# TorontoDeepLearning/convnet

Measured on AMD Instinct MI355X. Metric: images/sec (fprop+bprop+wgrad) AlexNet 224x224 bs=256, higher is better.
Workload: dtype f32

## Files before the change

convnet_amd/csrc/fewc_conv.hip:

```cpp
#include <algorithm>

#include "gather_gemm.h"

namespace chip {
namespace gfc {

constexpr int KX = 7, KY = 7, CH = 3, S = 2, NR = CH * KY, P = 4, IMG = 32;
constexpr int PW = S * (P - 1) + KX;
constexpr int XB = IMG * 4;
constexpr int RP = 2;
constexpr int ROWB = RP * 1024;
static_assert(PW * XB <= ROWB, "patch row");
constexpr int NCH = 10, ROWS = 96;
constexpr int H0_ROWS = 11, H1_ROWS = 10;
constexpr int H0_BYTES = H0_ROWS * ROWB, H1_BYTES = H1_ROWS * ROWB;
constexpr int BIAS_OFF = 0, BIAS_BYTES = 512;
constexpr int A_OFF = BIAS_BYTES;
constexpr int A_CHUNK = 6 * ROWS * 16;
constexpr int A_BYTES = NCH * A_CHUNK;
constexpr int A_PIECES = A_BYTES / 1024;
constexpr int PATCH_OFF = A_OFF + A_BYTES;
constexpr int ZERO_OFF = PATCH_OFF + H0_BYTES + H1_BYTES;
constexpr int ZERO_BYTES = 1024 + 256;
constexpr int LDS_BYTES = ZERO_OFF + ZERO_BYTES;
static_assert(LDS_BYTES <= 160 * 1024, "LDS");
static_assert(A_BYTES % 1024 == 0, "filter bank in whole pieces");
constexpr int NGROUP = 3 * 4;
constexpr int DUMP_BYTES = 4096;

__host__ __device__ constexpr int row_off(int r) { return r < 10 ? r * ROWB : r == 20 ? 10 * ROWB : H0_BYTES + (r - 10) * ROWB; }
__host__ __device__ constexpr int slot_k(int c, int lh, int j) {
  const int r = 2 * c + (j >> 2), kx = 2 * (j & 3) + lh;
  if (kx < KX) return kx + KX * r;
  return r < KX ? r + KX * 20 : -1;
}

struct Params {
  const float* src;
  const u32x4* planes;
  float* dst;
  float* dump;
  const float* bias;
  const float* zero;
  int F, N, H, W, My, Mx, pady, padx;
  int XG, IB, tiles;
  int relu;
  int diag;
};

}

__global__ void gfc_planes_kernel(const float* __restrict__ W, u32x4* __restrict__ out, int F) {
  using namespace gfc;
  const int i = blockIdx.x * blockDim.x + threadIdx.x;
  if (i >= NCH * 2 * ROWS) return;
  const int f = i % ROWS, lh = (i / ROWS) & 1, c = i / (2 * ROWS);
  Split8 sp = {};
  if (f < F) {
    float x[8];
#pragma unroll
    for (int j = 0; j < 8; ++j) {
      const int k = slot_k(c, lh, j);
      x[j] = k >= 0 ? W[(size_t)f + (size_t)F * k] : 0.f;
    }
    split8_sat(x, sp);
  }
  u32x4* o = out + ((size_t)c * 6 + lh) * ROWS + f;
  o[0] = sp.h;
  o[2 * ROWS] = sp.m;
  o[4 * ROWS] = sp.l;
}

template <bool RELU>
__global__ __launch_bounds__(320, 1) void gfc_kernel(const gfc::Params p) {
  using namespace gfc;
  extern __shared__ __attribute__((aligned(16))) float smem[];
  char* const lds = reinterpret_cast<char*>(smem);
  const int tid = threadIdx.x;
  const int wave = __builtin_amdgcn_readfirstlane(tid >> 6), lane = tid & 63;
  const int N = p.N;

  const int G = gridDim.x, q = p.tiles / G, rem = p.tiles % G, b = blockIdx.x;
  const int T0 = b * q + min(b, rem), T1 = T0 + q + (b < rem ? 1 : 0);
  if (T0 >= T1) return;
  int xg = T0 % p.XG, oy = (T0 / p.XG) % p.My, ib = T0 / (p.XG * p.My);
  auto next_tile = [&]() __attribute__((always_inline)) {
    if (++xg == p.XG) {
      xg = 0;
      if (++oy == p.My) {
        oy = 0;
        ++ib;
      }
    }
  };

  for (int i = wave; i < A_PIECES; i += 5) {
    const char* g = reinterpret_cast<const char*>(p.planes) + (size_t)i * 1024 + lane * 16;
    __builtin_amdgcn_global_load_lds((gbl_ptr_t)g, (lds_ptr_t)(lds + A_OFF + i * 1024), 16, 0, 0);
  }
  if (tid * 16 < ZERO_BYTES) *reinterpret_cast<u32x4*>(lds + ZERO_OFF + tid * 16) = u32x4{0, 0, 0, 0};
  if (tid < BIAS_BYTES / 4) *reinterpret_cast<float*>(lds + BIAS_OFF + tid * 4) = p.bias && tid < p.F ? p.bias[tid] : 0.f;

  if (wave == 4) {
    const int lx = lane >> 3;
    const unsigned lane_off = (unsigned)lx * (unsigned)(N * 4) + (unsigned)(lane & 7) * 16u;
    const size_t plane = (size_t)p.H * p.W * N * 4, rowb = (size_t)p.W * N * 4;
    auto issue_half = [&](auto HH) __attribute__((always_inline)) {
      constexpr int h = decltype(HH)::value;
      constexpr int n = h ? H1_ROWS : H0_ROWS;
      const int y0 = S * oy - p.pady, x0 = S * P * xg - p.padx;
      const char* const origin = reinterpret_cast<const char*>(p.src) + ((ptrdiff_t)y0 * p.W + x0) * (ptrdiff_t)(N * 4) + (ptrdiff_t)ib * (IMG * 4);
      bool xok[RP];
#pragma unroll
      for (int k = 0; k < RP; ++k) xok[k] = 8 * k + lx < PW && (unsigned)(x0 + 8 * k + lx) < (unsigned)p.W;
#pragma unroll
      for (int idx = 0; idx < n; ++idx) {
        const int r = h ? 10 + idx : idx == 10 ? 20 : idx;
        const int ch = r / KY, ky = r % KY;
        const bool yok = (unsigned)(y0 + ky) < (unsigned)p.H;
        const char* const rowp = origin + (size_t)ch * plane + (size_t)ky * rowb;
#pragma unroll
        for (int k = 0; k < RP; ++k) {
          const char* g = yok && xok[k] ? rowp + (size_t)(8 * k) * (size_t)(N * 4) + lane_off : reinterpret_cast<const char*>(p.zero);
          __builtin_amdgcn_global_load_lds((gbl_ptr_t)g, (lds_ptr_t)(lds + PATCH_OFF + (h ? H0_BYTES : 0) + idx * ROWB + k * 1024), 16, 0, 0);
        }
      }
    };
    using H0 = std::integral_constant<int, 0>;
    using H1 = std::integral_constant<int, 1>;
    issue_half(H0{});
    issue_half(H1{});
    __builtin_amdgcn_s_waitcnt(0x0070);
    __syncthreads();
    for (int T = T0; T < T1; ++T) {
      const bool more = T + 1 < T1 && !(p.diag & 2);
      __builtin_amdgcn_s_waitcnt(0x0070);
      __syncthreads();
      next_tile();
      if (more) issue_half(H0{});
      __builtin_amdgcn_s_waitcnt(0x0070);
      __syncthreads();
      if (more) issue_half(H1{});
    }
    __builtin_amdgcn_s_waitcnt(0x0070);
    return;
  }

  const int li = lane & 31, lh = lane >> 5;
  const unsigned base_l = (unsigned)(PATCH_OFF + (S * wave) * XB + li * 4 + lh * XB);
  const unsigned a_l = (unsigned)(A_OFF + (lh * ROWS + li) * 16);
  const unsigned lh_mask = lh ? 0xFFFFFFFFu : 0u;

  f32x16 acc[2][3];
  u32x4 fah[2][3], fam[3], fal[3];
  Split8 fb[2];
  float bv[8];
#ifndef CONVNET_EMU
#define CHIP_HERE() asm volatile("" ::: "memory")
#else
#define CHIP_HERE() ((void)0)
#endif
  auto read_a = [&](auto CC, auto PL, u32x4 (&dst)[3]) __attribute__((always_inline)) {
    constexpr int c = decltype(CC)::value, pl = decltype(PL)::value;
    CHIP_HERE();
#pragma unroll
    for (int t = 0; t < 3; ++t) dst[t] = *reinterpret_cast<const u32x4*>(lds + a_l + c * A_CHUNK + pl * (2 * ROWS * 16) + t * 512);
  };
  auto read_b = [&](auto CC) __attribute__((always_inline)) {
    constexpr int c = decltype(CC)::value;
    unsigned lhm = lh_mask;
    CHIP_HERE();
#ifndef CONVNET_EMU
    asm volatile("" : "+v"(lhm));
#endif
#pragma unroll
    for (int j = 0; j < 8; ++j) {
      const int r = 2 * c + (j >> 2);
      const int imm_n = row_off(r) + 2 * (j & 3) * XB;
      if ((j & 3) != 3) {
        bv[j] = *reinterpret_cast<const float*>(lds + base_l + imm_n);
      } else {
        const int imm_s = r < KX ? row_off(20) + (r - 1) * XB : (ZERO_OFF - PATCH_OFF);
        bv[j] = *reinterpret_cast<const float*>(lds + (base_l + (lhm & (unsigned)(imm_s - imm_n))) + imm_n);
      }
    }
  };
  auto split_pair = [&](int s, int q) __attribute__((always_inline)) {
    const float x0 = bv[2 * q], x1 = bv[2 * q + 1];
    const unsigned H = pk_bf16(x0, x1);
    const float r0 = x0 - __uint_as_float(H << 16), r1 = x1 - __uint_as_float(H & 0xffff0000u);
    const unsigned M = pk_bf16(r0, r1);
    const float s0 = r0 - __uint_as_float(M << 16), s1 = r1 - __uint_as_float(M & 0xffff0000u);
    fb[s].h[q] = H;
    fb[s].m[q] = M;
    fb[s].l[q] = pk_bf16(s0, s1);
#ifndef CONVNET_EMU
    asm volatile("" ::"v"(fb[s].h[q]), "v"(fb[s].m[q]), "v"(fb[s].l[q]));
#endif
  };
  auto mac_step = [&](auto K, int s, f32x16 (&a)[3]) __attribute__((always_inline)) {
    constexpr int k = decltype(K)::value;
#pragma unroll
    for (int t = 0; t < 3; ++t) {
      const u32x4& av = k == 1 ? fal[t] : k == 2 || k == 3 ? fam[t] : fah[s][t];
      const u32x4& bw = k == 0 ? fb[s].l : k == 2 || k == 4 ? fb[s].m : fb[s].h;
      a[t] = mma_bf16(av, bw, a[t]);
    }
#ifndef CONVNET_EMU
    asm volatile("" : "+v"(a[0]), "+v"(a[1]), "+v"(a[2]));
#endif
  };

  struct Out {
    unsigned lane_bytes;
    int flim;
  };
  const size_t fstride = (size_t)p.My * p.Mx * N;
  const int q4 = li & 3;
  auto out_of = [&](int xg_, int oy_, int ib_, bool exists) __attribute__((always_inline)) {
    const int ox = P * xg_ + wave;
    Out o;
    o.lane_bytes = (unsigned)((((size_t)oy_ * p.Mx + ox) * N + ib_ * IMG + 4 * (li >> 2) + (size_t)(q4 + 4 * lh) * fstride) * 4);
    o.flim = exists && ox < p.Mx ? p.F : 0;
#ifdef CONVNET_DIAG
    if (p.diag & 1) o.flim = 0;
#endif
    return o;
  };
  const unsigned bias_q = (unsigned)(BIAS_OFF + (q4 + 4 * lh) * 4);
  auto bias_of = [&](auto GG) __attribute__((always_inline)) {
    constexpr int gi = decltype(GG)::value;
    return *reinterpret_cast<const float*>(lds + bias_q + (32 * (gi >> 2) + 8 * (gi & 3)) * 4);
  };
  auto swap1 = [](float v) __attribute__((always_inline)) {
#ifndef CONVNET_EMU
    return __builtin_bit_cast(float, __builtin_amdgcn_mov_dpp(__builtin_bit_cast(int, v), 0xB1, 0xF, 0xF, true));
#else
    return emu::shfl_xor(v, 1);
#endif
  };
  auto swap2 = [](float v) __attribute__((always_inline)) {
#ifndef CONVNET_EMU
    return __builtin_bit_cast(float, __builtin_amdgcn_mov_dpp(__builtin_bit_cast(int, v), 0x4E, 0xF, 0xF, true));
#else
    return emu::shfl_xor(v, 2);
#endif
  };
  const bool odd1 = (li & 1) != 0, odd2 = (li & 2) != 0;
  auto store_group = [&](auto GG, const Out& o, const f32x16 (&a)[3], float bias) __attribute__((always_inline)) {
    constexpr int gi = decltype(GG)::value, t = gi >> 2, g = gi & 3;
    constexpr int cf = 32 * t + 8 * g;
    float x0 = a[t][4 * g], x1 = a[t][4 * g + 1], x2 = a[t][4 * g + 2], x3 = a[t][4 * g + 3];
    {
      const float r01 = swap1(odd1 ? x0 : x1), r23 = swap1(odd1 ? x2 : x3);
      x0 = odd1 ? r01 : x0; x1 = odd1 ? x1 : r01;
      x2 = odd1 ? r23 : x2; x3 = odd1 ? x3 : r23;
    }
    {
      const float ra = swap2(odd2 ? x0 : x2), rb = swap2(odd2 ? x1 : x3);
      x0 = odd2 ? ra : x0; x1 = odd2 ? rb : x1;
      x2 = odd2 ? x2 : ra; x3 = odd2 ? x3 : rb;
    }
    f32x4 v = {x0 + bias, x1 + bias, x2 + bias, x3 + bias};
    if constexpr (RELU) {
#pragma unroll
      for (int e = 0; e < 4; ++e) v[e] = fmaxf(v[e], 0.f);
    }
    const bool real = cf < o.flim;
    char* const rowb = real ? reinterpret_cast<char*>(p.dst) + (size_t)cf * fstride * 4 : reinterpret_cast<char*>(p.dump);
    const unsigned off = real ? o.lane_bytes : (unsigned)lane * 16u;
#ifdef CONVNET_DIAG
    if (p.diag & 4) return;
#endif
    *reinterpret_cast<f32x4*>(rowb + off) = v;
  };

  auto chunk_body = [&](auto CC, bool has_next, f32x16 (&cur)[3], const f32x16 (&prev)[3], const Out& po) __attribute__((always_inline)) {
    constexpr int c = decltype(CC)::value, s = c & 1;
    using CN = std::integral_constant<int, (c + 1) % NCH>;
    __builtin_amdgcn_sched_barrier(0);
    if (has_next) {
      read_b(CN{});
      read_a(CN{}, std::integral_constant<int, 0>{}, fah[s ^ 1]);
    }
    CHIP_HERE();
    const float bs0 = bias_of(std::integral_constant<int, c>{});
    float bs1 = 0.f;
    if constexpr (c >= 8) bs1 = bias_of(std::integral_constant<int, c + 2>{});
    static_for<0, 6>([&](auto KK) __attribute__((always_inline)) {
      constexpr int k = decltype(KK)::value;
      if constexpr (k >= 1 && k <= 4) {
        if (has_next) split_pair(s ^ 1, k - 1);
      }
      if constexpr (k == 0 && c >= 8) store_group(std::integral_constant<int, c + 2>{}, po, prev, bs1);
      if constexpr (k == 5) store_group(std::integral_constant<int, c>{}, po, prev, bs0);
      if constexpr (k == 2) {
        if (has_next) read_a(CN{}, std::integral_constant<int, 2>{}, fal);
      }
      if constexpr (k == 4) {
        if (has_next) read_a(CN{}, std::integral_constant<int, 1>{}, fam);
      }
      mac_step(KK, s, cur);
#pragma unroll
      for (int i = 0; i < 3; ++i) {
        __builtin_amdgcn_sched_group_barrier(0x008, 1, 0);
        __builtin_amdgcn_sched_group_barrier(0x100, 4, 0);
        __builtin_amdgcn_sched_group_barrier(0x002, 12, 0);
        __builtin_amdgcn_sched_group_barrier(0x040, 1, 0);
      }
      __builtin_amdgcn_sched_barrier(0);
    });
  };
  auto run_tile = [&](bool more, f32x16 (&cur)[3], const f32x16 (&prev)[3], const Out& po) __attribute__((always_inline)) {
#pragma unroll
    for (int t = 0; t < 3; ++t)
#pragma unroll
      for (int e = 0; e < 16; ++e) cur[t][e] = 0.f;
    static_for<0, NCH>([&](auto CC) __attribute__((always_inline)) {
      constexpr int c = decltype(CC)::value;
      if constexpr (c == 4) __syncthreads();
      if constexpr (c == NCH - 1) __syncthreads();
      if constexpr (c + 1 < NCH) chunk_body(CC, true, cur, prev, po);
      else chunk_body(CC, more, cur, prev, po);
    });
  };

  __builtin_amdgcn_s_waitcnt(0x0070);
  __syncthreads();
  {
    using C0 = std::integral_constant<int, 0>;
    read_b(C0{});
    read_a(C0{}, std::integral_constant<int, 0>{}, fah[0]);
    read_a(C0{}, std::integral_constant<int, 1>{}, fam);
    read_a(C0{}, std::integral_constant<int, 2>{}, fal);
  }
#pragma unroll
  for (int q4 = 0; q4 < 4; ++q4) split_pair(0, q4);
  Out po = out_of(0, 0, 0, false);
  int T = T0;
  for (;;) {
    run_tile(T + 1 < T1, acc[0], acc[1], po);
    po = out_of(xg, oy, ib, true);
    next_tile();
    if (++T >= T1) {
      static_for<0, NGROUP>([&](auto GG) __attribute__((always_inline)) { store_group(GG, po, acc[0], bias_of(GG)); });
      break;
    }
    run_tile(T + 1 < T1, acc[1], acc[0], po);
    po = out_of(xg, oy, ib, true);
    next_tile();
    if (++T >= T1) {
      static_for<0, NGROUP>([&](auto GG) __attribute__((always_inline)) { store_group(GG, po, acc[1], bias_of(GG)); });
      break;
    }
  }
}

bool gfc_try(const float* images, const float* filters, const float* bias, float* targets, int N, int C, int H, int W, int F, int Ky, int Kx,
             int sy, int sx, int pady, int padx, int My, int Mx, float scaleTargets, int relu, double flops) {
  using namespace gfc;
  if (!CHIP_KNOB("CONVNET_GG_FEWC", 1) || matrix_path() != 1) return false;
  if (Kx != KX || Ky != KY || C != CH || sy != S || sx != S || F > ROWS || F < 8 || F % 8 != 0 || N % IMG != 0 || My < 1 || Mx < 1) return false;
  if (pady < 0 || padx < 0 || (size_t)C * H * W * N * 4 >= (size_t(1) << 32) || (size_t)F * My * Mx * N * 4 >= (size_t(1) << 32)) return false;
  if (scaleTargets != 0.f) return false;
  if ((reinterpret_cast<uintptr_t>(images) | reinterpret_cast<uintptr_t>(targets)) & 15) return false;
  static bool once = false;
  static int cus = 256;
  if (!once) {
    CHIP_CHECK(hipFuncSetAttribute(reinterpret_cast<const void*>(gfc_kernel<false>), hipFuncAttributeMaxDynamicSharedMemorySize, LDS_BYTES));
    CHIP_CHECK(hipFuncSetAttribute(reinterpret_cast<const void*>(gfc_kernel<true>), hipFuncAttributeMaxDynamicSharedMemorySize, LDS_BYTES));
#ifndef CONVNET_EMU
    int dev = 0;
    hipDeviceProp_t prop;
    if (hipGetDevice(&dev) == hipSuccess && hipGetDeviceProperties(&prop, dev) == hipSuccess && prop.multiProcessorCount > 0) cus = prop.multiProcessorCount;
#else
    cus = 4;
#endif
    once = true;
  }
  u32x4* planes = static_cast<u32x4*>(workspace_aux(A_BYTES + DUMP_BYTES));
  (void)filter_planes_shared(nullptr, 0);
  {
    KernelTimer timer("filter_planes_kernel", "conv_fprop", 0.0, 4.0 * F * C * Ky * Kx + A_BYTES);
    hipLaunchKernelGGL(gfc_planes_kernel, dim3(divup(NCH * 2 * ROWS, 256)), dim3(256), 0, stream(), filters, planes, F);
  }
  Params p{};
  p.src = images; p.planes = planes; p.dst = targets; p.bias = bias; p.zero = zero_page();
  p.dump = reinterpret_cast<float*>(reinterpret_cast<char*>(planes) + A_BYTES);
  p.F = F; p.N = N; p.H = H; p.W = W; p.My = My; p.Mx = Mx; p.pady = pady; p.padx = padx;
  p.XG = divup(Mx, P); p.IB = N / IMG; p.tiles = p.XG * My * p.IB;
  p.relu = relu; p.diag = CHIP_DIAG_KNOB("CONVNET_GFC_DIAG", 0);
  const int grid = std::min(cus, p.tiles);
  {
    KernelTimer timer("gfc_kernel<96x128,split>", "conv_fprop", flops, 0.0, 0.0);
    if (relu) hipLaunchKernelGGL(gfc_kernel<true>, dim3(grid), dim3(320), LDS_BYTES, stream(), p);
    else hipLaunchKernelGGL(gfc_kernel<false>, dim3(grid), dim3(320), LDS_BYTES, stream(), p);
  }
  note_kernel("gfc_kernel(fprop)", flops, grid, 1);
  return true;
}

}
```

Baseline: 27920.

## Add wide 8-pixel tile variant for first-layer conv with shared producer loads

Adds a WIDE variant of the few-channel 7x7 stride-2 conv kernel in which each wave computes two output pixels, so there are 8 per tile instead of 4. Overlapping input columns are reused by shifting the already-split bf16 halves rather than re-splitting them. The dedicated producer wave is removed; all four compute waves share the patch refill and wait on vmcnt so that stores can stay in flight. Accumulators are pinned to AGPRs and the first MMA starts from a zero accumulator. The wide path is chosen when there are at least four tiles per CU, which costs more LDS and register pressure.

Measured after the change: 28000 (median of 3 runs). No clear change (+0.3%).

```diff
diff --git a/convnet_amd/csrc/fewc_conv.hip b/convnet_amd/csrc/fewc_conv.hip
--- a/convnet_amd/csrc/fewc_conv.hip
+++ b/convnet_amd/csrc/fewc_conv.hip
@@ -5,30 +5,48 @@
 namespace chip {
 namespace gfc {
 
-constexpr int KX = 7, KY = 7, CH = 3, S = 2, NR = CH * KY, P = 4, IMG = 32;
-constexpr int PW = S * (P - 1) + KX;
+constexpr int KX = 7, KY = 7, CH = 3, S = 2, NR = CH * KY, IMG = 32;
 constexpr int XB = IMG * 4;
-constexpr int RP = 2;
-constexpr int ROWB = RP * 1024;
-static_assert(PW * XB <= ROWB, "patch row");
 constexpr int NCH = 10, ROWS = 96;
 constexpr int H0_ROWS = 11, H1_ROWS = 10;
-constexpr int H0_BYTES = H0_ROWS * ROWB, H1_BYTES = H1_ROWS * ROWB;
 constexpr int BIAS_OFF = 0, BIAS_BYTES = 512;
 constexpr int A_OFF = BIAS_BYTES;
 constexpr int A_CHUNK = 6 * ROWS * 16;
 constexpr int A_BYTES = NCH * A_CHUNK;
 constexpr int A_PIECES = A_BYTES / 1024;
 constexpr int PATCH_OFF = A_OFF + A_BYTES;
-constexpr int ZERO_OFF = PATCH_OFF + H0_BYTES + H1_BYTES;
 constexpr int ZERO_BYTES = 1024 + 256;
-constexpr int LDS_BYTES = ZERO_OFF + ZERO_BYTES;
-static_assert(LDS_BYTES <= 160 * 1024, "LDS");
 static_assert(A_BYTES % 1024 == 0, "filter bank in whole pieces");
-constexpr int NGROUP = 3 * 4;
 constexpr int DUMP_BYTES = 4096;
 
-__host__ __device__ constexpr int row_off(int r) { return r < 10 ? r * ROWB : r == 20 ? 10 * ROWB : H0_BYTES + (r - 10) * ROWB; }
+template <bool WIDE>
+struct Tile {
+  static constexpr int P = WIDE ? 8 : 4;
+  static constexpr int PPW = P / 4;
+  static constexpr int PW = S * (P - 1) + KX;
+  static constexpr int RP = WIDE ? 3 : 2;
+  static constexpr int ROWB = RP * 1024;
+  static constexpr int H0_BYTES = H0_ROWS * ROWB, H1_BYTES = H1_ROWS * ROWB;
+  static constexpr int ZERO_OFF = PATCH_OFF + H0_BYTES + H1_BYTES;
+  static constexpr int LDS_BYTES = ZERO_OFF + ZERO_BYTES;
+  static constexpr int THREADS = WIDE ? 256 : 320;
+  static constexpr int NACC = 3 * PPW;
+  static constexpr int NGROUP = 4 * NACC;
+  static_assert(PW * XB <= ROWB, "patch row");
+  static_assert(LDS_BYTES <= 160 * 1024, "LDS");
+  static_assert((WIDE ? 0 : S * 3 * XB) + (PPW - 1) * S * XB + XB + IMG * 4 <= ZERO_BYTES, "zero region");
+  __host__ __device__ static constexpr int row_off(int r) { return r < 10 ? r * ROWB : r == 20 ? 10 * ROWB : H0_BYTES + (r - 10) * ROWB; }
+};
+__host__ __device__ constexpr int wide_extra(int c) { return c == 1 ? 0 : c == 3 ? 1 : c == 6 ? 2 : c == 8 ? 3 : -1; }
+__host__ __device__ constexpr int wide_stores(int c0, int n) {
+  int s = 0;
+  for (int i = 0; i < n; ++i) s += 2 + (wide_extra((c0 + i) % NCH) >= 0 ? 1 : 0);
+  return s;
+}
+static_assert(wide_stores(0, NCH) == Tile<true>::NGROUP, "every group of the previous tile leaves during this one");
+constexpr int WIDE_STORES_IN_FLIGHT = wide_stores(4, 5);
+static_assert(wide_stores(9, 5) == WIDE_STORES_IN_FLIGHT && WIDE_STORES_IN_FLIGHT < 16, "one vmcnt immediate for both refill waits");
+
 __host__ __device__ constexpr int slot_k(int c, int lh, int j) {
   const int r = 2 * c + (j >> 2), kx = 2 * (j & 3) + lh;
   if (kx < KX) return kx + KX * r;
@@ -71,9 +89,12 @@
   o[4 * ROWS] = sp.l;
 }
 
-template <bool RELU>
-__global__ __launch_bounds__(320, 1) void gfc_kernel(const gfc::Params p) {
+template <bool RELU, bool WIDE>
+__global__ __launch_bounds__(gfc::Tile<WIDE>::THREADS, 1) void gfc_kernel(const gfc::Params p) {
   using namespace gfc;
+  using TL = Tile<WIDE>;
+  constexpr int P = TL::P, PPW = TL::PPW, PW = TL::PW, RP = TL::RP, ROWB = TL::ROWB, H0_BYTES = TL::H0_BYTES, ZERO_OFF = TL::ZERO_OFF;
+  constexpr int NACC = TL::NACC, NGROUP = TL::NGROUP, NW = TL::THREADS / 64;
   extern __shared__ __attribute__((aligned(16))) float smem[];
   char* const lds = reinterpret_cast<char*>(smem);
   const int tid = threadIdx.x;
@@ -94,67 +115,131 @@
     }
   };
 
-  for (int i = wave; i < A_PIECES; i += 5) {
+  for (int i = wave; i < A_PIECES; i += NW) {
     const char* g = reinterpret_cast<const char*>(p.planes) + (size_t)i * 1024 + lane * 16;
     __builtin_amdgcn_global_load_lds((gbl_ptr_t)g, (lds_ptr_t)(lds + A_OFF + i * 1024), 16, 0, 0);
   }
   if (tid * 16 < ZERO_BYTES) *reinterpret_cast<u32x4*>(lds + ZERO_OFF + tid * 16) = u32x4{0, 0, 0, 0};
   if (tid < BIAS_BYTES / 4) *reinterpret_cast<float*>(lds + BIAS_OFF + tid * 4) = p.bias && tid < p.F ? p.bias[tid] : 0.f;
 
-  if (wave == 4) {
-    const int lx = lane >> 3;
-    const unsigned lane_off = (unsigned)lx * (unsigned)(N * 4) + (unsigned)(lane & 7) * 16u;
-    const size_t plane = (size_t)p.H * p.W * N * 4, rowb = (size_t)p.W * N * 4;
-    auto issue_half = [&](auto HH) __attribute__((always_inline)) {
-      constexpr int h = decltype(HH)::value;
-      constexpr int n = h ? H1_ROWS : H0_ROWS;
-      const int y0 = S * oy - p.pady, x0 = S * P * xg - p.padx;
-      const char* const origin = reinterpret_cast<const char*>(p.src) + ((ptrdiff_t)y0 * p.W + x0) * (ptrdiff_t)(N * 4) + (ptrdiff_t)ib * (IMG * 4);
-      bool xok[RP];
-#pragma unroll
-      for (int k = 0; k < RP; ++k) xok[k] = 8 * k + lx < PW && (unsigned)(x0 + 8 * k + lx) < (unsigned)p.W;
-#pragma unroll
-      for (int idx = 0; idx < n; ++idx) {
-        const int r = h ? 10 + idx : idx == 10 ? 20 : idx;
-        const int ch = r / KY, ky = r % KY;
-        const bool yok = (unsigned)(y0 + ky) < (unsigned)p.H;
-        const char* const rowp = origin + (size_t)ch * plane + (size_t)ky * rowb;
-#pragma unroll
-        for (int k = 0; k < RP; ++k) {
-          const char* g = yok && xok[k] ? rowp + (size_t)(8 * k) * (size_t)(N * 4) + lane_off : reinterpret_cast<const char*>(p.zero);
-          __builtin_amdgcn_global_load_lds((gbl_ptr_t)g, (lds_ptr_t)(lds + PATCH_OFF + (h ? H0_BYTES : 0) + idx * ROWB + k * 1024), 16, 0, 0);
-        }
-      }
-    };
-    using H0 = std::integral_constant<int, 0>;
-    using H1 = std::integral_constant<int, 1>;
-    issue_half(H0{});
-    issue_half(H1{});
-    __builtin_amdgcn_s_waitcnt(0x0070);
-    __syncthreads();
-    for (int T = T0; T < T1; ++T) {
-      const bool more = T + 1 < T1 && !(p.diag & 2);
+  const int lx = lane >> 3;
+  const unsigned lane_off = (unsigned)lx * (unsigned)(N * 4) + (unsigned)(lane & 7) * 16u;
+  const size_t plane = (size_t)p.H * p.W * N * 4, rowb = (size_t)p.W * N * 4;
+  struct RowSrc {
+    size_t rel;
+    int ky;
+  };
+  auto row_src = [&](int h, int idx) __attribute__((always_inline)) {
+    const int r = h ? 10 + idx : idx == 10 ? 20 : idx;
+    const int ch = r / KY, ky = r % KY;
+    return RowSrc{(size_t)ch * plane + (size_t)ky * rowb, ky};
+  };
+  struct Origin {
+    const char* at;
+    int y0;
+    bool xok[RP];
+  };
+  auto origin_of = [&](int xg_, int oy_, int ib_) __attribute__((always_inline)) {
+    Origin o;
+    const int x0 = S * P * xg_ - p.padx;
+    o.y0 = S * oy_ - p.pady;
+    o.at = reinterpret_cast<const char*>(p.src) + ((ptrdiff_t)o.y0 * p.W + x0) * (ptrdiff_t)(N * 4) + (ptrdiff_t)ib_ * (IMG * 4);
+#pragma unroll
+    for (int k = 0; k < RP; ++k) o.xok[k] = 8 * k + lx < PW && (unsigned)(x0 + 8 * k + lx) < (unsigned)p.W;
+    return o;
+  };
+  auto issue_row = [&](auto HH, int idx, const RowSrc& rs, const Origin& o) __attribute__((always_inline)) {
+    constexpr int h = decltype(HH)::value;
+    const bool yok = (unsigned)(o.y0 + rs.ky) < (unsigned)p.H;
+    const char* const rowp = o.at + rs.rel;
+#pragma unroll
+    for (int k = 0; k < RP; ++k) {
+      const char* g = yok && o.xok[k] ? rowp + (size_t)(8 * k) * (size_t)(N * 4) + lane_off : reinterpret_cast<const char*>(p.zero);
+      __builtin_amdgcn_global_load_lds((gbl_ptr_t)g, (lds_ptr_t)(lds + PATCH_OFF + (h ? H0_BYTES : 0) + idx * ROWB + k * 1024), 16, 0, 0);
+    }
+  };
+  using H0 = std::integral_constant<int, 0>;
+  using H1 = std::integral_constant<int, 1>;
+
+  if constexpr (!WIDE) {
+    if (wave == 4) {
+      auto issue_half = [&](auto HH) __attribute__((always_inline)) {
+        constexpr int h = decltype(HH)::value;
+        const Origin o = origin_of(xg, oy, ib);
+#pragma unroll
+        for (int idx = 0; idx < (h ? H1_ROWS : H0_ROWS); ++idx) issue_row(HH, idx, row_src(h, idx), o);
+      };
+      issue_half(H0{});
+      issue_half(H1{});
       __builtin_amdgcn_s_waitcnt(0x0070);
       __syncthreads();
-      next_tile();
-      if (more) issue_half(H0{});
+      for (int T = T0; T < T1; ++T) {
+        const bool more = T + 1 < T1 && !(p.diag & 2);
+        __builtin_amdgcn_s_waitcnt(0x0070);
+        __syncthreads();
+        next_tile();
+        if (more) issue_half(H0{});
+        __builtin_amdgcn_s_waitcnt(0x0070);
+        __syncthreads();
+        if (more) issue_half(H1{});
+      }
       __builtin_amdgcn_s_waitcnt(0x0070);
-      __syncthreads();
-      if (more) issue_half(H1{});
-    }
-    __builtin_amdgcn_s_waitcnt(0x0070);
-    return;
+      return;
+    }
+  }
+  constexpr int NSHARE = 3;
+  static_assert(!WIDE || (4 * NSHARE >= H0_ROWS && 4 * (NSHARE - 1) < H1_ROWS), "rows of a half over four waves");
+  RowSrc share_src[2][NSHARE];
+  if constexpr (WIDE) {
+#pragma unroll
+    for (int h = 0; h < 2; ++h)
+#pragma unroll
+      for (int m = 0; m < NSHARE; ++m) share_src[h][m] = row_src(h, min(wave + 4 * m, (h ? H1_ROWS : H0_ROWS) - 1));
+  }
+  auto issue_share = [&](auto HH, int xg_, int oy_, int ib_) __attribute__((always_inline)) {
+    constexpr int h = decltype(HH)::value;
+    const Origin o = origin_of(xg_, oy_, ib_);
+#pragma unroll
+    for (int m = 0; m < NSHARE; ++m) {
+      const int idx = wave + 4 * m;
+      if (m + 1 < NSHARE || idx < (h ? H1_ROWS : H0_ROWS)) issue_row(HH, idx, share_src[h][m], o);
+    }
+  };
+  int nxg = 0, noy = 0, nib = 0;
+  auto peek_next = [&]() __attribute__((always_inline)) {
+    nxg = xg; noy = oy; nib = ib;
+    if (++nxg == p.XG) {
+      nxg = 0;
+      if (++noy == p.My) {
+        noy = 0;
+        ++nib;
+      }
+    }
+  };
+  auto wait_refill = [&]() __attribute__((always_inline)) {
+#ifdef CONVNET_DIAG
+    if (p.diag & 4) {
+      __builtin_amdgcn_s_waitcnt(0x0070);
+      return;
+    }
+#endif
+    __builtin_amdgcn_s_waitcnt(0x0070 | WIDE_STORES_IN_FLIGHT);
+  };
+  if constexpr (WIDE) {
+    issue_share(H0{}, xg, oy, ib);
+    issue_share(H1{}, xg, oy, ib);
   }
 
   const int li = lane & 31, lh = lane >> 5;
-  const unsigned base_l = (unsigned)(PATCH_OFF + (S * wave) * XB + li * 4 + lh * XB);
+  const unsigned base_l = (unsigned)(PATCH_OFF + (S * PPW * wave) * XB + li * 4 + lh * XB);
   const unsigned a_l = (unsigned)(A_OFF + (lh * ROWS + li) * 16);
   const unsigned lh_mask = lh ? 0xFFFFFFFFu : 0u;
-
-  f32x16 acc[2][3];
+  const unsigned zero_rel = (unsigned)(ZERO_OFF - PATCH_OFF) - (unsigned)((S * PPW * wave) * XB);
+
+  f32x16 acc[2][NACC];
   u32x4 fah[2][3], fam[3], fal[3];
-  Split8 fb[2];
-  float bv[8];
+  Split8 fb[2][PPW];
+  float bv[PPW][8];
 #ifndef CONVNET_EMU
 #define CHIP_HERE() asm volatile("" ::: "memory")
 #else
@@ -176,60 +261,92 @@
 #pragma unroll
     for (int j = 0; j < 8; ++j) {
       const int r = 2 * c + (j >> 2);
-      const int imm_n = row_off(r) + 2 * (j & 3) * XB;
-      if ((j & 3) != 3) {
-        bv[j] = *reinterpret_cast<const float*>(lds + base_l + imm_n);
-      } else {
-        const int imm_s = r < KX ? row_off(20) + (r - 1) * XB : (ZERO_OFF - PATCH_OFF);
-        bv[j] = *reinterpret_cast<const float*>(lds + (base_l + (lhm & (unsigned)(imm_s - imm_n))) + imm_n);
-      }
-    }
-  };
-  auto split_pair = [&](int s, int q) __attribute__((always_inline)) {
-    const float x0 = bv[2 * q], x1 = bv[2 * q + 1];
+      const int imm_n = TL::row_off(r) + 2 * (j & 3) * XB;
+      unsigned at = base_l;
+      if ((j & 3) == 3) {
+        if (WIDE && r >= KX) {
+          at = base_l + (lhm & (zero_rel - (unsigned)imm_n));
+        } else {
+          const int imm_s = r < KX ? TL::row_off(20) + (r - 1) * XB : (ZERO_OFF - PATCH_OFF);
+          at = base_l + (lhm & (unsigned)(imm_s - imm_n));
+        }
+      }
+#pragma unroll
+      for (int px = 0; px < PPW; ++px)
+        if (px == 0 || (j & 3) >= 2) bv[px][j] = *reinterpret_cast<const float*>(lds + at + imm_n + px * (S * XB));
+    }
+  };
+  auto split_pair = [&](int s, int px, int q) __attribute__((always_inline)) {
+    if (px > 0 && (q & 1) == 0) {
+      const Split8& f0 = fb[s][px - 1];
+      Split8& f = fb[s][px];
+      f.h[q] = (f0.h[q] >> 16) | (f0.h[q + 1] << 16);
+      f.m[q] = (f0.m[q] >> 16) | (f0.m[q + 1] << 16);
+      f.l[q] = (f0.l[q] >> 16) | (f0.l[q + 1] << 16);
+#ifndef CONVNET_EMU
+      asm volatile("" ::"v"(f.h[q]), "v"(f.m[q]), "v"(f.l[q]));
+#endif
+      return;
+    }
+    const float x0 = bv[px][2 * q], x1 = bv[px][2 * q + 1];
     const unsigned H = pk_bf16(x0, x1);
     const float r0 = x0 - __uint_as_float(H << 16), r1 = x1 - __uint_as_float(H & 0xffff0000u);
     const unsigned M = pk_bf16(r0, r1);
     const float s0 = r0 - __uint_as_float(M << 16), s1 = r1 - __uint_as_float(M & 0xffff0000u);
-    fb[s].h[q] = H;
-    fb[s].m[q] = M;
-    fb[s].l[q] = pk_bf16(s0, s1);
-#ifndef CONVNET_EMU
-    asm volatile("" ::"v"(fb[s].h[q]), "v"(fb[s].m[q]), "v"(fb[s].l[q]));
-#endif
-  };
-  auto mac_step = [&](auto K, int s, f32x16 (&a)[3]) __attribute__((always_inline)) {
+    Split8& f = fb[s][px];
+    f.h[q] = H;
+    f.m[q] = M;
+    f.l[q] = pk_bf16(s0, s1);
+#ifndef CONVNET_EMU
+    asm volatile("" ::"v"(f.h[q]), "v"(f.m[q]), "v"(f.l[q]));
+#endif
+  };
+  auto mac_step = [&](auto K, auto FIRST, int s, f32x16 (&a)[NACC]) __attribute__((always_inline)) {
     constexpr int k = decltype(K)::value;
-#pragma unroll
-    for (int t = 0; t < 3; ++t) {
-      const u32x4& av = k == 1 ? fal[t] : k == 2 || k == 3 ? fam[t] : fah[s][t];
-      const u32x4& bw = k == 0 ? fb[s].l : k == 2 || k == 4 ? fb[s].m : fb[s].h;
-      a[t] = mma_bf16(av, bw, a[t]);
-    }
-#ifndef CONVNET_EMU
-    asm volatile("" : "+v"(a[0]), "+v"(a[1]), "+v"(a[2]));
+    constexpr bool first = decltype(FIRST)::value;
+#pragma unroll
+    for (int px = 0; px < PPW; ++px) {
+#pragma unroll
+      for (int t = 0; t < 3; ++t) {
+        const u32x4& av = k == 1 ? fal[t] : k == 2 || k == 3 ? fam[t] : fah[s][t];
+        const Split8& f = fb[s][px];
+        const u32x4& bw = k == 0 ? f.l : k == 2 || k == 4 ? f.m : f.h;
+        if constexpr (first) {
+          const f32x16 zero = {0.f, 0.f, 0.f, 0.f, 0.f, 0.f, 0.f, 0.f, 0.f, 0.f, 0.f, 0.f, 0.f, 0.f, 0.f, 0.f};
+          a[3 * px + t] = mma_bf16(av, bw, zero);
+        } else {
+          a[3 * px + t] = mma_bf16(av, bw, a[3 * px + t]);
+        }
+      }
+    }
+#ifndef CONVNET_EMU
+    if constexpr (WIDE) asm volatile("" : "+a"(a[0]), "+a"(a[1]), "+a"(a[2]), "+a"(a[3]), "+a"(a[4]), "+a"(a[5]));
+    else asm volatile("" : "+v"(a[0]), "+v"(a[1]), "+v"(a[2]));
 #endif
   };
 
   struct Out {
-    unsigned lane_bytes;
-    int flim;
+    unsigned lane_bytes[PPW];
+    int flim[PPW];
   };
   const size_t fstride = (size_t)p.My * p.Mx * N;
   const int q4 = li & 3;
   auto out_of = [&](int xg_, int oy_, int ib_, bool exists) __attribute__((always_inline)) {
-    const int ox = P * xg_ + wave;
     Out o;
-    o.lane_bytes = (unsigned)((((size_t)oy_ * p.Mx + ox) * N + ib_ * IMG + 4 * (li >> 2) + (size_t)(q4 + 4 * lh) * fstride) * 4);
-    o.flim = exists && ox < p.Mx ? p.F : 0;
+#pragma unroll
+    for (int px = 0; px < PPW; ++px) {
+      const int ox = P * xg_ + PPW * wave + px;
+      o.lane_bytes[px] = (unsigned)((((size_t)oy_ * p.Mx + ox) * N + ib_ * IMG + 4 * (li >> 2) + (size_t)(q4 + 4 * lh) * fstride) * 4);
+      o.flim[px] = exists && ox < p.Mx ? p.F : 0;
 #ifdef CONVNET_DIAG
-    if (p.diag & 1) o.flim = 0;
-#endif
+      if (p.diag & 1) o.flim[px] = 0;
+#endif
+    }
     return o;
   };
   const unsigned bias_q = (unsigned)(BIAS_OFF + (q4 + 4 * lh) * 4);
   auto bias_of = [&](auto GG) __attribute__((always_inline)) {
-    constexpr int gi = decltype(GG)::value;
+    constexpr int gi = decltype(GG)::value % 12;
     return *reinterpret_cast<const float*>(lds + bias_q + (32 * (gi >> 2) + 8 * (gi & 3)) * 4);
   };
   auto swap1 = [](float v) __attribute__((always_inline)) {
@@ -247,10 +364,11 @@
 #endif
   };
   const bool odd1 = (li & 1) != 0, odd2 = (li & 2) != 0;
-  auto store_group = [&](auto GG, const Out& o, const f32x16 (&a)[3], float bias) __attribute__((always_inline)) {
-    constexpr int gi = decltype(GG)::value, t = gi >> 2, g = gi & 3;
+  auto store_group = [&](auto GG, const Out& o, const f32x16 (&a)[NACC], float bias) __attribute__((always_inline)) {
+    constexpr int gi = decltype(GG)::value, px = gi / 12, t = (gi % 12) >> 2, g = gi & 3;
     constexpr int cf = 32 * t + 8 * g;
-    float x0 = a[t][4 * g], x1 = a[t][4 * g + 1], x2 = a[t][4 * g + 2], x3 = a[t][4 * g + 3];
+    const f32x16& at = a[3 * px + t];
+    float x0 = acc_elem<WIDE>(at[4 * g]), x1 = acc_elem<WIDE>(at[4 * g + 1]), x2 = acc_elem<WIDE>(at[4 * g + 2]), x3 = acc_elem<WIDE>(at[4 * g + 3]);
     {
       const float r01 = swap1(odd1 ? x0 : x1), r23 = swap1(odd1 ? x2 : x3);
       x0 = odd1 ? r01 : x0; x1 = odd1 ? x1 : r01;
@@ -266,16 +384,16 @@
 #pragma unroll
       for (int e = 0; e < 4; ++e) v[e] = fmaxf(v[e], 0.f);
     }
-    const bool real = cf < o.flim;
+    const bool real = cf < o.flim[px];
     char* const rowb = real ? reinterpret_cast<char*>(p.dst) + (size_t)cf * fstride * 4 : reinterpret_cast<char*>(p.dump);
-    const unsigned off = real ? o.lane_bytes : (unsigned)lane * 16u;
+    const unsigned off = real ? o.lane_bytes[px] : (unsigned)lane * 16u;
 #ifdef CONVNET_DIAG
     if (p.diag & 4) return;
 #endif
     *reinterpret_cast<f32x4*>(rowb + off) = v;
   };
 
-  auto chunk_body = [&](auto CC, bool has_next, f32x16 (&cur)[3], const f32x16 (&prev)[3], const Out& po) __attribute__((always_inline)) {
+  auto chunk_body = [&](auto CC, bool has_next, f32x16 (&cur)[NACC], const f32x16 (&prev)[NACC], const Out& po) __attribute__((always_inline)) {
     constexpr int c = decltype(CC)::value, s = c & 1;
     using CN = std::integral_constant<int, (c + 1) % NCH>;
     __builtin_amdgcn_sched_barrier(0);
@@ -284,42 +402,75 @@
       read_a(CN{}, std::integral_constant<int, 0>{}, fah[s ^ 1]);
     }
     CHIP_HERE();
-    const float bs0 = bias_of(std::integral_constant<int, c>{});
-    float bs1 = 0.f;
-    if constexpr (c >= 8) bs1 = bias_of(std::integral_constant<int, c + 2>{});
+    constexpr int G0 = WIDE ? (wide_extra(c) >= 0 ? 2 * NCH + wide_extra(c) : -1) : (c >= 8 ? c + 2 : -1);
+    constexpr int G3 = WIDE ? 2 * c : -1, G5 = WIDE ? 2 * c + 1 : c;
+    const float bs5 = bias_of(std::integral_constant<int, G5>{});
+    float bs0 = 0.f, bs3 = 0.f;
+    if constexpr (G0 >= 0) bs0 = bias_of(std::integral_constant<int, G0>{});
+    if constexpr (G3 >= 0) bs3 = bias_of(std::integral_constant<int, G3>{});
     static_for<0, 6>([&](auto KK) __attribute__((always_inline)) {
       constexpr int k = decltype(KK)::value;
-      if constexpr (k >= 1 && k <= 4) {
-        if (has_next) split_pair(s ^ 1, k - 1);
-      }
-      if constexpr (k == 0 && c >= 8) store_group(std::integral_constant<int, c + 2>{}, po, prev, bs1);
-      if constexpr (k == 5) store_group(std::integral_constant<int, c>{}, po, prev, bs0);
+      if constexpr (!WIDE) {
+        if constexpr (k >= 1 && k <= 4) {
+          if (has_next) split_pair(s ^ 1, 0, k - 1);
+        }
+      } else {
+        constexpr int i0 = k == 1 ? 0 : k == 2 ? 3 : k == 4 ? 6 : 8, i1 = k == 1 ? 3 : k == 2 ? 6 : 8;
+        if (has_next) {
+#pragma unroll
+          for (int i = i0; i < i1; ++i) split_pair(s ^ 1, i >> 2, i & 3);
+        }
+      }
+      if constexpr (k == 0 && G0 >= 0) store_group(std::integral_constant<int, (G0 >= 0 ? G0 : 0)>{}, po, prev, bs0);
+      if constexpr (k == 3 && G3 >= 0) store_group(std::integral_constant<int, (G3 >= 0 ? G3 : 0)>{}, po, prev, bs3);
+      if constexpr (k == 5) store_group(std::integral_constant<int, G5>{}, po, prev, bs5);
       if constexpr (k == 2) {
         if (has_next) read_a(CN{}, std::integral_constant<int, 2>{}, fal);
       }
       if constexpr (k == 4) {
         if (has_next) read_a(CN{}, std::integral_constant<int, 1>{}, fam);
       }
-      mac_step(KK, s, cur);
-#pragma unroll
-      for (int i = 0; i < 3; ++i) {
+      mac_step(KK, std::bool_constant<WIDE && c == 0 && k == 0>{}, s, cur);
+#pragma unroll
+      for (int i = 0; i < NACC; ++i) {
         __builtin_amdgcn_sched_group_barrier(0x008, 1, 0);
         __builtin_amdgcn_sched_group_barrier(0x100, 4, 0);
-        __builtin_amdgcn_sched_group_barrier(0x002, 12, 0);
+        __builtin_amdgcn_sched_group_barrier(0x002, WIDE ? 8 : 12, 0);
         __builtin_amdgcn_sched_group_barrier(0x040, 1, 0);
       }
       __builtin_amdgcn_sched_barrier(0);
     });
   };
-  auto run_tile = [&](bool more, f32x16 (&cur)[3], const f32x16 (&prev)[3], const Out& po) __attribute__((always_inline)) {
-#pragma unroll
-    for (int t = 0; t < 3; ++t)
-#pragma unroll
-      for (int e = 0; e < 16; ++e) cur[t][e] = 0.f;
+  auto run_tile = [&](bool more, f32x16 (&cur)[NACC], const f32x16 (&prev)[NACC], const Out& po) __attribute__((always_inline)) {
+    if constexpr (!WIDE) {
+#pragma unroll
+      for (int t = 0; t < 3; ++t)
+#pragma unroll
+        for (int e = 0; e < 16; ++e) cur[t][e] = 0.f;
+    }
+    const bool refill = more && !(p.diag & 2);
     static_for<0, NCH>([&](auto CC) __attribute__((always_inline)) {
       constexpr int c = decltype(CC)::value;
-      if constexpr (c == 4) __syncthreads();
-      if constexpr (c == NCH - 1) __syncthreads();
+      if constexpr (c == 4 || c == NCH - 1) {
+        if constexpr (WIDE) {
+          __builtin_amdgcn_sched_barrier(0);
+          wait_refill();
+          CHIP_HERE();
+          __builtin_amdgcn_s_barrier();
+          CHIP_HERE();
+        } else {
+          __syncthreads();
+        }
+        if constexpr (WIDE) {
+          CHIP_HERE();
+          if (c == 4) peek_next();
+          if (refill) {
+            if constexpr (c == 4) issue_share(H0{}, nxg, noy, nib);
+            else issue_share(H1{}, nxg, noy, nib);
+          }
+          CHIP_HERE();
+        }
+      }
       if constexpr (c + 1 < NCH) chunk_body(CC, true, cur, prev, po);
       else chunk_body(CC, more, cur, prev, po);
     });
@@ -335,7 +486,9 @@
     read_a(C0{}, std::integral_constant<int, 2>{}, fal);
   }
 #pragma unroll
-  for (int q4 = 0; q4 < 4; ++q4) split_pair(0, q4);
+  for (int px = 0; px < PPW; ++px)
+#pragma unroll
+    for (int q = 0; q < 4; ++q) split_pair(0, px, q);
   Out po = out_of(0, 0, 0, false);
   int T = T0;
   for (;;) {
@@ -343,6 +496,7 @@
     po = out_of(xg, oy, ib, true);
     next_tile();
     if (++T >= T1) {
+      if constexpr (WIDE) acc_settle();
       static_for<0, NGROUP>([&](auto GG) __attribute__((always_inline)) { store_group(GG, po, acc[0], bias_of(GG)); });
       break;
     }
@@ -350,10 +504,18 @@
     po = out_of(xg, oy, ib, true);
     next_tile();
     if (++T >= T1) {
+      if constexpr (WIDE) acc_settle();
       static_for<0, NGROUP>([&](auto GG) __attribute__((always_inline)) { store_group(GG, po, acc[1], bias_of(GG)); });
       break;
     }
   }
+}
+
+template <bool WIDE>
+static void gfc_launch(const gfc::Params& p, int grid) {
+  using TL = gfc::Tile<WIDE>;
+  if (p.relu) hipLaunchKernelGGL((gfc_kernel<true, WIDE>), dim3(grid), dim3(TL::THREADS), TL::LDS_BYTES, stream(), p);
+  else hipLaunchKernelGGL((gfc_kernel<false, WIDE>), dim3(grid), dim3(TL::THREADS), TL::LDS_BYTES, stream(), p);
 }
 
 bool gfc_try(const float* images, const float* filters, const float* bias, float* targets, int N, int C, int H, int W, int F, int Ky, int Kx,
@@ -367,8 +529,10 @@
   static bool once = false;
   static int cus = 256;
   if (!once) {
-    CHIP_CHECK(hipFuncSetAttribute(reinterpret_cast<const void*>(gfc_kernel<false>), hipFuncAttributeMaxDynamicSharedMemorySize, LDS_BYTES));
-    CHIP_CHECK(hipFuncSetAttribute(reinterpret_cast<const void*>(gfc_kernel<true>), hipFuncAttributeMaxDynamicSharedMemorySize, LDS_BYTES));
+    CHIP_CHECK(hipFuncSetAttribute(reinterpret_cast<const void*>(gfc_kernel<false, false>), hipFuncAttributeMaxDynamicSharedMemorySize, Tile<false>::LDS_BYTES));
+    CHIP_CHECK(hipFuncSetAttribute(reinterpret_cast<const void*>(gfc_kernel<true, false>), hipFuncAttributeMaxDynamicSharedMemorySize, Tile<false>::LDS_BYTES));
+    CHIP_CHECK(hipFuncSetAttribute(reinterpret_cast<const void*>(gfc_kernel<false, true>), hipFuncAttributeMaxDynamicSharedMemorySize, Tile<true>::LDS_BYTES));
+    CHIP_CHECK(hipFuncSetAttribute(reinterpret_cast<const void*>(gfc_kernel<true, true>), hipFuncAttributeMaxDynamicSharedMemorySize, Tile<true>::LDS_BYTES));
 #ifndef CONVNET_EMU
     int dev = 0;
     hipDeviceProp_t prop;
@@ -388,13 +552,17 @@
   p.src = images; p.planes = planes; p.dst = targets; p.bias = bias; p.zero = zero_page();
   p.dump = reinterpret_cast<float*>(reinterpret_cast<char*>(planes) + A_BYTES);
   p.F = F; p.N = N; p.H = H; p.W = W; p.My = My; p.Mx = Mx; p.pady = pady; p.padx = padx;
-  p.XG = divup(Mx, P); p.IB = N / IMG; p.tiles = p.XG * My * p.IB;
+  const int wide_tiles = divup(Mx, Tile<true>::P) * My * (N / IMG);
+  const bool wide = wide_tiles >= 4 * cus;
+  p.XG = divup(Mx, wide ? Tile<true>::P : Tile<false>::P); p.IB = N / IMG; p.tiles = p.XG * My * p.IB;
   p.relu = relu; p.diag = CHIP_DIAG_KNOB("CONVNET_GFC_DIAG", 0);
   const int grid = std::min(cus, p.tiles);
-  {
+  if (wide) {
+    KernelTimer timer("gfc_kernel<96x256,split>", "conv_fprop", flops, 0.0, 0.0);
+    gfc_launch<true>(p, grid);
+  } else {
     KernelTimer timer("gfc_kernel<96x128,split>", "conv_fprop", flops, 0.0, 0.0);
-    if (relu) hipLaunchKernelGGL(gfc_kernel<true>, dim3(grid), dim3(320), LDS_BYTES, stream(), p);
-    else hipLaunchKernelGGL(gfc_kernel<false>, dim3(grid), dim3(320), LDS_BYTES, stream(), p);
+    gfc_launch<false>(p, grid);
   }
   note_kernel("gfc_kernel(fprop)", flops, grid, 1);
   return true;
```
